# lanl-ansi/Katana.jl

Hardware: AMD Instinct MI355X
Metric: ECP iterations/sec + wall-clock to f_tol=1e-6, 1e5-var synthetic convex NLP (higher is better)
Workload: dtype f64; 1 GPU; cfg3: n=100000 variables, m_lin=50000 linear rows (8 nnz), m_nl=10000 explog rows (k=32 nnz), seed 0, planted non-degenerate vertex optimum, f_tol=1e-6; parallelism=1 GPU

## Files before the change

katana.jl_amd/csrc/engine.hpp:

```cpp
#pragma once
#include <hip/hip_runtime.h>

#include <algorithm>
#include <chrono>
#include <cstdlib>
#include <cmath>
#include <limits>
#include <map>
#include <string>
#include <vector>

#include <rccl/rccl.h>

#include "common.hpp"
#include "types.hpp"
#include "prims.hpp"

namespace ktn {

static const double kInf = std::numeric_limits<double>::infinity();

static inline int pick_group(double avg_len) {
    int g = 4;
    while (g < 64 && 2 * g <= avg_len) g <<= 1;
// ... 169 lines not shown
    void append_link(int64_t nrows, const int64_t* nl_id_host);
    void append_link_dev(int64_t nrows);
    int64_t* list_heads() { return glists ? d_glast.p : d_lastcut.p; }
    int64_t list_count() const { return glists ? nl_total : m_nl; }
    bool lists_ok() const { return !sharded_rows || glists; }
    DBuf<int64_t> c_ptr, c_cnt;
    DBuf<int32_t> c_row;
    DBuf<double> c_val, c_sval, r_sval;
    DBuf<uint32_t> c_perm, c_perm2;
    DBuf<int32_t> c_row2;
    DBuf<int64_t> c_ptr2, c_off;
    int64_t csc_M = -1, csc_NNZ = 0;
    uint64_t lp_epoch = 1, csc_epoch = 0;
    void csc_merge_appended();
    bool w_shift = false;
    int64_t M_lin = 0;
    DBuf<double> wval, wlo, whi, wc, epi_ref, epi_scal;
    DBuf<unsigned long long> epi_newest;
    const double* Wval() const { return w_shift ? wval.p : lp_val.p; }
    const double* Wlo() const { return w_shift ? wlo.p : lp_lo.p; }
    const double* Whi() const { return w_shift ? whi.p : lp_hi.p; }
    const double* Wc() const { return w_shift ? wc.p : lp_c.p; }
    bool want_shift(int mode) const { return prm.epi_shift != 0 && !obj_linear && mode == 0 && !row_sharded() && n_blocks == 0; }
    void build_working();
    void ensure_matrix(bool shift);
    void epi_dot(const double* x);
    DBuf<uint64_t> k_in, k_out;
    DBuf<uint32_t> p_in, p_out;
    DBuf<char> d_sorttmp;
    DBuf<double> dr_r, dc_r;
    DBuf<ColRec> d_crec;
    DBuf<RowRec> d_rrec;
    DBuf<int2> d_cbl;
    bool packed_on = false;
    int packed_trips = 1;
    DBuf<double> dr2, dc2;
    DBuf<double> dr, dc, statr, statc, ch, lh, uh, loh, hih, xh, yh, x0h, y0h, xth, yth, xbar, pv, pw, box;
    DBuf<double> partials, chk_part, chkout, power_v, power_v0;
    int64_t power_v0_n = -1;
    double* h_chk = nullptr;
    double* h_chk_dev = nullptr;
    int64_t lp_iter_budget = 0, dense_credit = 0, dense_run = 0;
    DBuf<int32_t> ds_W, ds_valid;
    DBuf<double> ds_dense, ds_out;
    DBuf<double> md_Binv, md_hW, md_x, md_lam, md_u, md_d, md_r, md_pv, md_c, md_aug, md_prow, md_fcol;
    int64_t md_since_refactor = 0;
    DBuf<double> md_y;
    uint64_t md_y_version = 0;
    bool mid_true_duals(double* y_out);
    int64_t mid_backoff = 0, mid_backoff_len = 0;
    DBuf<int32_t> md_W, md_pi, md_lost;
    DBuf<MidState> md_st;
    bool md_valid = false;
    int64_t mid_credit = 0, mid_run = 0;
    DBuf<int32_t> d_longrows;
    DBuf<int32_t> d_longcols;
    int64_t n_longc = 0;
    int64_t col_gain_max = 0;
    int64_t col_len_max = -1, col_scan_rows = 0;
    int64_t col_removed_rows = 0;
    void find_long_cols();
    void spmv_cols(const SpMat& AT, const double* v, double* out, hipEvent_t e0 = nullptr, hipEvent_t e1 = nullptr);
    static constexpr int kMaxChunk = 512;
    int64_t n_long = 0;
    static constexpr int64_t kLongRow = 2048;
    int64_t max_row_len = (int64_t)1 << 62;
// ... 310 lines not shown
```

katana.jl_amd/csrc/kernels.hpp:

```cpp
#pragma once
#include <hip/hip_runtime.h>

#include <cstdint>
#include <type_traits>

#include "../../include/katana_hip.h"
#include "types.hpp"

namespace ktn {

constexpr int kKindShift = 29;
constexpr int kColMask = (1 << kKindShift) - 1;

template <int G>
__device__ __forceinline__ double group_sum(double v) {
#pragma unroll
    for (int off = G / 2; off > 0; off >>= 1) v += __shfl_xor(v, off, 64);
    return v;
}
template <int G>
__device__ __forceinline__ double group_max(double v) {
#pragma unroll
    for (int off = G / 2; off > 0; off >>= 1) v = fmax(v, __shfl_xor(v, off, 64));
    return v;
// ... 674 lines not shown
                                                     const int32_t* __restrict__ col, const double* __restrict__ jac,
                                                     const double* __restrict__ g, const double* __restrict__ lb, const double* __restrict__ ub,
                                                     const int64_t* __restrict__ lp_rowptr, int32_t* __restrict__ lp_col,
                                                     double* __restrict__ lp_val, double* __restrict__ lp_lo, double* __restrict__ lp_hi) {
    const int64_t r = (int64_t)blockIdx.x * kBlock + threadIdx.x;
    if (r >= nlin) return;
    const int32_t i = lin_rows[r];
    const int64_t beg = rowptr[i], len = rowptr[i + 1] - beg, dst = lp_rowptr[r];
    double b = g[i];
    for (int64_t e = 0; e < len; ++e) {
        const double jv = jac[beg + e];
        lp_col[dst + e] = col[beg + e];
        lp_val[dst + e] = jv;
        b += -0.0 * jv;
    }
    lp_lo[r] = lb[i] - b;
    lp_hi[r] = ub[i] - b;
}

struct LpRows {
    int64_t* rowptr;
    int32_t* col;
    double* val;
    double* lo;
    double* hi;
    double* y;
};

static __global__ __launch_bounds__(kBlock) void k_compact(NlpDev P, const int32_t* __restrict__ nl_rows, int64_t m_nl,
                                                    const int64_t* __restrict__ flag, const int64_t* __restrict__ rank,
                                                    const int64_t* __restrict__ cnt_scan, const double* __restrict__ bconst,
                                                    int64_t base_row, int64_t base_nnz, LpRows L,
                                                    int32_t* __restrict__ viol_slots, int64_t* __restrict__ last_cut,
                                                    int64_t* __restrict__ cut_prev, int inherit) {
    const int64_t gid = (int64_t)blockIdx.x * kBlock + threadIdx.x;
    if (gid >= m_nl) return;
    if (!flag[gid]) return;
    const int32_t r = nl_rows[gid];
    const int64_t v = rank[gid];
    const int64_t R = base_row + v;
    const int64_t len = P.rowptr[r + 1] - P.rowptr[r];
    L.rowptr[R + 1] = base_nnz + cnt_scan[gid] + len;
    const double b = bconst[r];
    L.lo[R] = P.lb[r] - b;
    L.hi[R] = P.ub[r] - b;
    viol_slots[v] = (int32_t)gid;
    double y0 = 0.0;
    const int64_t prev = last_cut[gid];
    if (inherit && prev >= 0) { y0 = L.y[prev]; L.y[prev] = 0.0; }
    L.y[R] = y0;
    cut_prev[R] = prev;
    last_cut[gid] = R;
}

static __global__ __launch_bounds__(kBlock) void k_append_link(int64_t nrows, int64_t base_row, const int64_t* __restrict__ nl_id,
                                                       int64_t nl_total, int64_t* __restrict__ glast,
                                                       int64_t* __restrict__ cut_prev, double* __restrict__ y, int inherit) {
    const int64_t i = (int64_t)blockIdx.x * kBlock + threadIdx.x;
    if (i >= nrows) return;
    const int64_t R = base_row + i, g = nl_id[i];
    double y0 = 0.0;
    int64_t prev = -1;
    if (g >= 0 && g < nl_total) {
        prev = glast[g];
        if (inherit && prev >= 0) { y0 = y[prev]; y[prev] = 0.0; }
        glast[g] = R;
    }
    y[R] = y0;
    cut_prev[R] = prev;
}

static __global__ __launch_bounds__(kBlock) void k_consolidate(int64_t m_nl, const int64_t* __restrict__ last_cut,
                                                        const int64_t* __restrict__ cut_prev, const double* __restrict__ ax,
                                                        const double* __restrict__ lo, const double* __restrict__ hi,
                                                        const double* __restrict__ dr, double thresh,
                                                        double* __restrict__ y, int32_t* __restrict__ moved) {
    const int64_t s = (int64_t)blockIdx.x * kBlock + threadIdx.x;
    if (s >= m_nl) return;
    int64_t best_u = -1, best_l = -1;
    double res_u = -__builtin_inf(), res_l = -__builtin_inf();
    int ncuts = 0;
    for (int64_t r = last_cut[s]; r >= 0; r = cut_prev[r]) {
        ++ncuts;
        const double ru = ax[r] - hi[r], rl = lo[r] - ax[r];
        if (ru > res_u) { res_u = ru; best_u = r; }
// ... 175 lines not shown
};
constexpr unsigned kChkRowMask = 0x141Fu;
constexpr unsigned kChkColMask = 0x6FE0u;
template <int BLOCK, unsigned MASK, int G = 1>
__device__ __forceinline__ void chk_block_store(ChkAcc& a, double* partials) {
    __shared__ double sh[kChkQ][BLOCK / 64];
    const int lane = threadIdx.x & 63, wv = threadIdx.x >> 6;
#pragma unroll
    for (int off = 32; off >= G; off >>= 1) {
#pragma unroll
        for (int q = 0; q < kChkQ; ++q) {
            if (!((MASK >> q) & 1u)) continue;
            const double o = __shfl_xor(a.s[q], off, 64);
            a.s[q] = (q < 12) ? a.s[q] + o : fmax(a.s[q], o);
        }
    }
    if (lane == 0) {
#pragma unroll
        for (int q = 0; q < kChkQ; ++q)
            if ((MASK >> q) & 1u) sh[q][wv] = a.s[q];
    }
    __syncthreads();
    if (threadIdx.x < kChkQ) {
        const int q = threadIdx.x;
        double v = 0.0;
        if ((MASK >> q) & 1u) {
            v = sh[q][0];
            for (int k = 1; k < BLOCK / 64; ++k) v = (q < 12) ? v + sh[q][k] : fmax(v, sh[q][k]);
        }
        partials[(int64_t)blockIdx.x * kChkQ + q] = v;
    }
}

template <int G, bool UPDATE>
__global__ __launch_bounds__(kBlock) void k_pdhg_x(int64_t n, SpMat AT, const double* __restrict__ y,
                                                   double* __restrict__ x, const double* __restrict__ x0,
                                                   double* __restrict__ xt, double* __restrict__ xbar,
                                                   const double* __restrict__ c, const double* __restrict__ l,
                                                   const double* __restrict__ u, double tau, double w, double rho) {
    const int64_t j = ((int64_t)blockIdx.x * kBlock + threadIdx.x) / G;
    const int lane = threadIdx.x & (G - 1);
    if (j >= n) return;
    const int64_t beg = AT.ptr[j], end = AT.ptr[j + 1];
    const double xv = x[j], cj = c[j], lj = l[j], uj = u[j], x0j = (UPDATE || xbar) ? x0[j] : 0.0;
    double acc = 0.0;
    for (int64_t e = beg + lane; e < end; e += G) acc += AT.val[e] * y[AT.idx[e]];
    acc = group_sum<G>(acc);
    if (lane == 0) {
        const double xtv = prox_x(xv, tau, cj, acc, lj, uj);
        if (UPDATE) { xbar[j] = 2.0 * xtv - xv; x[j] = halpern(w, rho, xtv, xv, x0j); }
        else {
            xt[j] = xtv;
            if (xbar) xbar[j] = halpern(w, rho, xtv, xv, x0j);
        }
    }
}

template <int G, bool UPDATE>
__global__ __launch_bounds__(kBlock) void k_pdhg_x_skip(int64_t n, SpMat AT, const double* __restrict__ y,
                                                        double* __restrict__ x, const double* __restrict__ x0,
                                                        double* __restrict__ xt, double* __restrict__ xbar,
                                                        const double* __restrict__ c, const double* __restrict__ l,
                                                        const double* __restrict__ u, double tau, double w, double rho, int64_t skip_longer) {
    const int64_t j = ((int64_t)blockIdx.x * kBlock + threadIdx.x) / G;
    const int lane = threadIdx.x & (G - 1);
    if (j >= n) return;
// ... 199 lines not shown
}

template <int G>
__global__ __launch_bounds__(kBlock) void k_pdhg_y_chk(int64_t m, SpMat A, const double* __restrict__ xt,
                                                       const double* __restrict__ x, const double* __restrict__ y,
                                                       const double* __restrict__ y0, double* __restrict__ yt,
                                                       const double* __restrict__ lo, const double* __restrict__ hi,
                                                       const double* __restrict__ dr, double sigma, int64_t long_thresh,
                                                       double* __restrict__ partials, double* __restrict__ ynext, double w, double rho) {
    const int64_t i = ((int64_t)blockIdx.x * kBlock + threadIdx.x) / G;
    const int lane = threadIdx.x & (G - 1);
    ChkAcc a; a.init();
    const bool on = i < m;
    const int64_t beg = on ? A.ptr[i] : 0, end = on ? A.ptr[i + 1] : 0;
    const bool mine = on && (end - beg <= long_thresh);
    double yv = 0.0, loi = 0.0, hii = 0.0, y0i = 0.0, dri = 1.0;
    if (mine) { yv = y[i]; loi = lo[i]; hii = hi[i]; y0i = y0[i]; dri = dr[i]; }
    double axt = 0.0, axk = 0.0;
    if (mine)
        for (int64_t e = beg + lane; e < end; e += G) {
            const int c = A.idx[e];
            const double v = A.val[e];
            axt += v * xt[c];
            axk += v * x[c];
        }
    axt = group_sum<G>(axt);
    axk = group_sum<G>(axk);
    if (mine && lane == 0) {
        const double ytv = prox_y(yv, sigma, 2.0 * axt - axk, loi, hii);
        yt[i] = ytv;
        if (ynext) ynext[i] = halpern(w, rho, ytv, yv, y0i);
        chk_row_accumulate(a, ytv, yv, y0i, axt, axk, loi, hii, dri);
    }
    chk_block_store<kBlock, kChkRowMask, G>(a, partials);
}

constexpr int kLongBlock = 1024;
template <bool CHECK>
__global__ __launch_bounds__(kLongBlock) void k_pdhg_y_long(const int32_t* __restrict__ rows, SpMat A,
                                                        const double* __restrict__ xa, const double* __restrict__ xb,
                                                        double* __restrict__ y, const double* __restrict__ y0,
                                                        double* __restrict__ yt, const double* __restrict__ lo,
                                                        const double* __restrict__ hi, const double* __restrict__ dr,
                                                        double sigma, double w, double rho, double* __restrict__ partials) {
    const int64_t i = rows[blockIdx.x];
    const int64_t beg = A.ptr[i], end = A.ptr[i + 1];
    double acc = 0.0, acc2 = 0.0;
    for (int64_t e = beg + threadIdx.x; e < end; e += kLongBlock) {
        const int c = A.idx[e];
        const double v = A.val[e];
        acc += v * xa[c];
        if (CHECK) acc2 += v * xb[c];
    }
    __shared__ double sh[2][kLongBlock / 64];
    double a2[2] = {acc, acc2};
    block_sum<kLongBlock>(a2, sh);
    if (threadIdx.x == 0) {
        const double ax = a2[0], ax2 = a2[1];
        const double yv = y[i];
        if (CHECK) {
            const double ytv = prox_y(yv, sigma, 2.0 * ax - ax2, lo[i], hi[i]);
            yt[i] = ytv;
            ChkAcc a; a.init();
            chk_row_accumulate(a, ytv, yv, y0[i], ax, ax2, lo[i], hi[i], dr[i]);
#pragma unroll
            for (int q = 0; q < kChkQ; ++q) partials[(int64_t)blockIdx.x * kChkQ + q] = a.s[q];
        } else {
// ... 82 lines not shown
}
__device__ __forceinline__ void chk_col_accumulate(ChkAcc& a, double xtv, double xv, double x0v, double aty, double cj, double lj,
                                                   double uj, double dcj) {
    const ChkColTerms t = chk_col_terms(xtv, xv, x0v, aty, cj, lj, uj, dcj);
    a.s[5] += t.dx2;
    a.s[6] += t.pobj;
    a.s[7] += t.dobj;
    a.s[8] += t.dx0sq;
    a.s[9] += t.xt2;
    a.s[13] = fmax(a.s[13], t.dres);
    const double r0 = -aty;
    if (r0 > 0.0) { if (isfinite(lj)) { a.s[10] += lj * r0; a.s[11] += fabs(lj * r0); } else a.s[14] = fmax(a.s[14], r0); }
    else if (r0 < 0.0) { if (isfinite(uj)) { a.s[10] += uj * r0; a.s[11] += fabs(uj * r0); } else a.s[14] = fmax(a.s[14], -r0); }
}
template <int G>
__global__ __launch_bounds__(kBlock) void k_chk_cols(int64_t n, SpMat AT, const double* __restrict__ x,
                                                     const double* __restrict__ xt, const double* __restrict__ x0,
                                                     const double* __restrict__ yt, const double* __restrict__ c,
                                                     const double* __restrict__ l, const double* __restrict__ u,
                                                     const double* __restrict__ dc, double* __restrict__ partials) {
    const int64_t j = ((int64_t)blockIdx.x * kBlock + threadIdx.x) / G;
    const int lane = threadIdx.x & (G - 1);
    ChkAcc a; a.init();
    const bool on = j < n;
    const int64_t beg = on ? AT.ptr[j] : 0, end = on ? AT.ptr[j + 1] : 0;
    double xtv = 0.0, xv = 0.0, x0v = 0.0, cj = 0.0, lj = 0.0, uj = 0.0, dcj = 1.0;
    if (on) { xtv = xt[j]; xv = x[j]; x0v = x0[j]; cj = c[j]; lj = l[j]; uj = u[j]; dcj = dc[j]; }
    double aty = 0.0;
    for (int64_t e = beg + lane; e < end; e += G) aty += AT.val[e] * yt[AT.idx[e]];
    aty = group_sum<G>(aty);
    if (on && lane == 0) {
        chk_col_accumulate(a, xtv, xv, x0v, aty, cj, lj, uj, dcj);
    }
    chk_block_store<kBlock, kChkColMask, G>(a, partials);
}

template <bool UPDATE>
__global__ __launch_bounds__(kBlock) void k_x_prox(int64_t n, const double* __restrict__ aty, double* __restrict__ x,
                                                   const double* __restrict__ x0, double* __restrict__ xt, double* __restrict__ xbar,
                                                   const double* __restrict__ c, const double* __restrict__ l,
                                                   const double* __restrict__ u, double tau, double w, double rho) {
    const int64_t j = (int64_t)blockIdx.x * kBlock + threadIdx.x;
    if (j >= n) return;
    const double xv = x[j];
    const double xtv = prox_x(xv, tau, c[j], aty[j], l[j], u[j]);
    if (UPDATE) { xbar[j] = 2.0 * xtv - xv; x[j] = halpern(w, rho, xtv, xv, x0[j]); }
    else xt[j] = xtv;
}
static __global__ __launch_bounds__(kBlock) void k_chk_cols_vec(int64_t n, const double* __restrict__ atyv, const double* __restrict__ x,
                                                         const double* __restrict__ xt, const double* __restrict__ x0,
                                                         const double* __restrict__ c, const double* __restrict__ l,
                                                         const double* __restrict__ u, const double* __restrict__ dc,
                                                         double* __restrict__ partials) {
    const int64_t j = (int64_t)blockIdx.x * kBlock + threadIdx.x;
    ChkAcc a; a.init();
    if (j < n) {
        const double xtv = xt[j], xv = x[j], x0v = x0[j], cj = c[j], lj = l[j], uj = u[j], dcj = dc[j], aty = atyv[j];
        chk_col_accumulate(a, xtv, xv, x0v, aty, cj, lj, uj, dcj);
    }
    chk_block_store<kBlock, kChkColMask>(a, partials);
}

__device__ __forceinline__ double ipc_load(const double* p) {
    return __longlong_as_double((long long)__hip_atomic_load((unsigned long long*)p, __ATOMIC_RELAXED, __HIP_MEMORY_SCOPE_SYSTEM));
}
static __global__ __launch_bounds__(64) void k_ipc_barrier(IpcPeers P, int rank, int world, unsigned long long epoch, long long timeout_ticks,
                                                    int* __restrict__ err) {
// ... 657 lines not shown
    if (i < n) out[i] = (s > 0.0) ? a[i] / sqrt(s) : 0.0;
}
static __global__ __launch_bounds__(kBlock) void k_fill(int64_t n, double* __restrict__ z, double v) {
    const int64_t i = (int64_t)blockIdx.x * kBlock + threadIdx.x;
    if (i < n) z[i] = v;
}
static __global__ __launch_bounds__(kBlock) void k_axpy_scaled(int64_t n, const double* __restrict__ a, double s, double* __restrict__ out) {
    const int64_t i = (int64_t)blockIdx.x * kBlock + threadIdx.x;
    if (i < n) out[i] = a[i] * s;
}

template <int G>
__global__ __launch_bounds__(kBlock) void k_csc_keys(int64_t m, const int64_t* __restrict__ rowptr,
                                                     const int32_t* __restrict__ col, uint64_t* __restrict__ keys,
                                                     uint32_t* __restrict__ vals, int64_t* __restrict__ colcount) {
    const int64_t i = ((int64_t)blockIdx.x * kBlock + threadIdx.x) / G;
    const int lane = threadIdx.x & (G - 1);
    if (i >= m) return;
    for (int64_t e = rowptr[i] + lane; e < rowptr[i + 1]; e += G) {
        const uint32_t c = (uint32_t)col[e];
        keys[e] = ((uint64_t)c << 32) | (uint64_t)(uint32_t)i;
        vals[e] = (uint32_t)e;
        atomicAdd(reinterpret_cast<unsigned long long*>(&colcount[c]), 1ULL);
    }
}
static __global__ __launch_bounds__(kBlock) void k_cscm_count(int64_t e0, int64_t nnz, const int32_t* __restrict__ col, int64_t* __restrict__ cnt) {
    const int64_t e = e0 + (int64_t)blockIdx.x * kBlock + threadIdx.x;
    if (e < nnz) atomicAdd(reinterpret_cast<unsigned long long*>(&cnt[col[e]]), 1ULL);
}
template <int G>
__global__ __launch_bounds__(kBlock) void k_cscm_move(int64_t n, const int64_t* __restrict__ old_ptr, const int64_t* __restrict__ off,
                                                      const int32_t* __restrict__ old_row, const uint32_t* __restrict__ old_perm,
                                                      int64_t* __restrict__ new_ptr, int32_t* __restrict__ new_row,
                                                      uint32_t* __restrict__ new_perm) {
    const int64_t j = ((int64_t)blockIdx.x * kBlock + threadIdx.x) / G;
    const int lane = threadIdx.x & (G - 1);
    if (j > n) return;
    if (j == n) { if (lane == 0) new_ptr[n] = old_ptr[n] + off[n]; return; }
    const int64_t src = old_ptr[j], len = old_ptr[j + 1] - src, dst = src + off[j];
    for (int64_t k = lane; k < len; k += G) { new_row[dst + k] = old_row[src + k]; new_perm[dst + k] = old_perm[src + k]; }
    if (lane == 0) new_ptr[j] = dst;
}
template <int G>
__global__ __launch_bounds__(kBlock) void k_cscm_place(int64_t m0, int64_t m, const int64_t* __restrict__ rowptr, const int32_t* __restrict__ col,
                                                       const int64_t* __restrict__ old_ptr, const int64_t* __restrict__ off,
                                                       int64_t* __restrict__ cursor, int32_t* __restrict__ new_row,
                                                       uint32_t* __restrict__ new_perm) {
    const int64_t r = m0 + ((int64_t)blockIdx.x * kBlock + threadIdx.x) / G;
    const int lane = threadIdx.x & (G - 1);
    if (r >= m) return;
    for (int64_t e = rowptr[r] + lane; e < rowptr[r + 1]; e += G) {
        const int32_t j = col[e];
        const int64_t k = (int64_t)atomicAdd(reinterpret_cast<unsigned long long*>(&cursor[j]), 1ULL);
        const int64_t pos = old_ptr[j + 1] + off[j] + k;
        new_row[pos] = (int32_t)r;
        new_perm[pos] = (uint32_t)e;
    }
}
static __global__ __launch_bounds__(kBlock) void k_cscm_order(int64_t n, const int64_t* __restrict__ old_ptr, const int64_t* __restrict__ off,
                                                       int32_t* __restrict__ new_row, uint32_t* __restrict__ new_perm) {
    const int64_t j = (int64_t)blockIdx.x * kBlock + threadIdx.x;
    if (j >= n) return;
    const int64_t cnt = off[j + 1] - off[j];
    if (cnt < 2) return;
    const int64_t b = old_ptr[j + 1] + off[j];
    for (int64_t a = 1; a < cnt; ++a) {
        const int32_t rr = new_row[b + a];
        const uint32_t pp = new_perm[b + a];
        int64_t q = a - 1;
        while (q >= 0 && (new_row[b + q] > rr || (new_row[b + q] == rr && new_perm[b + q] > pp))) {
// ... 213 lines not shown
```

katana.jl_amd/csrc/lp.hip:

```cpp
#include "engine.hpp"
#include "launch.hpp"
#include "kernels.hpp"
#include "pdhg_check.hpp"
#include "dense_lp.hpp"
#include "mid_lp.hpp"
#include "batch_lp.hpp"

namespace ktn {

double Engine::dev_dot(int64_t n, const double* a, const double* b) {
    hipLaunchKernelGGL(k_dot_partial, dim3(kRedBlocks), dim3(kBlock), 0, stream, n, a, b, partials.p);
    hipLaunchKernelGGL(k_sum_final, dim3(1), dim3(kRedBlocks), 0, stream, partials.p, kRedBlocks, chkout.p + 2 * kChkQ);
    double v = 0.0;
    KTN_HIP(hipMemcpyAsync(&v, chkout.p + 2 * kChkQ, sizeof(double), hipMemcpyDeviceToHost, stream));
    sync();
    return v;
}

double Engine::dev_finite_sq(int64_t n, const double* a) {
    hipLaunchKernelGGL(k_finite_sq_partial, dim3(kRedBlocks), dim3(kBlock), 0, stream, n, a, partials.p);
    hipLaunchKernelGGL(k_sum_final, dim3(1), dim3(kRedBlocks), 0, stream, partials.p, kRedBlocks, chkout.p + 2 * kChkQ);
    double v = 0.0;
    KTN_HIP(hipMemcpyAsync(&v, chkout.p + 2 * kChkQ, sizeof(double), hipMemcpyDeviceToHost, stream));
    sync();
// ... 310 lines not shown
    const bool tiled_chk_off = dev.no_tiled_check;
    if (tiled_on && m > 0 && !tiled_chk_off) {
        const int64_t brow_t = ceil_div(m, (int64_t)kBlock), bcol_t = ceil_div(n, (int64_t)kBlock);
        launch_tiled(tAT, n, m, yh.p, nullptr);
        if (row_sharded()) {
            LAUNCH_1(k_tile_vec, n, stream, n, tAT.pcnt.p, tpart.p, pv.p);
            allreduce(pv.p, (size_t)n, 0);
            LAUNCH_1(k_x_prox<false>, n, stream, n, pv.p, xh.p, x0h.p, xth.p, xbar.p, ch.p, lh.p, uh.p, tau, 0.0, 1.0);
        } else {
            LAUNCH_1(k_x_epilogue_chk, n, stream, n, tAT.pcnt.p, tpart.p, xh.p, xth.p, ch.p, lh.p, uh.p, tau);
        }
        launch_tiled(tA, m, n, xth.p, nullptr);
        LAUNCH_1(k_tile_vec, m, stream, m, tA.pcnt.p, tpart.p, pw.p);
        launch_tiled(tA, m, n, xh.p, nullptr);
        LAUNCH_1(k_y_epilogue_chk, m, stream, m, tA.pcnt.p, tpart.p, pw.p, (n_long > 0 ? A.ptr : (const int64_t*)nullptr), thr, yh.p, y0h.p,
                 yth.p, loh.p, hih.p, dr.p, sigma, prow);
        if (n_long > 0)
            hipLaunchKernelGGL((k_pdhg_y_long<true>), dim3((unsigned)n_long), dim3(kLongBlock), 0, stream, d_longrows.p, A, xth.p, xh.p,
                               yh.p, y0h.p, yth.p, loh.p, hih.p, dr.p, sigma, 0.0, 1.0, prow + (size_t)brow_t * kChkQ);
        chk_nrow = (int)(brow_t + n_long);
        launch_tiled(tAT, n, m, yth.p, nullptr);
        LAUNCH_1(k_tile_vec, n, stream, n, tAT.pcnt.p, tpart.p, pv.p);
        if (row_sharded()) allreduce(pv.p, (size_t)n, 0);
        LAUNCH_1(k_chk_cols_vec, n, stream, n, pv.p, xh.p, xth.p, x0h.p, ch.p, lh.p, uh.p, dc.p, pcol);
        chk_ncol = (int)bcol_t;
        hipLaunchKernelGGL(k_chk_final, dim3(2 * kChkQ), dim3(kRedBlocks), 0, stream, prow, chk_nrow, pcol, chk_ncol, chk_target());
        if (row_sharded()) {
            allreduce(chkout.p, 12, 0);
            allreduce(chkout.p + 12, 4, 1);
        }
        return false;
    }
    const bool spec = w_next >= 0.0 && m > 0 && !row_sharded() && n_long == 0 && n_longc == 0;
    if (spec) {
        xnext.resize((size_t)n, stream); ynext.resize((size_t)m, stream);
        LAUNCH_GB(grp_cols, k_pdhg_x, false, n, stream, n, AT, yh.p, xh.p, x0h.p, xth.p, xnext.p, ch.p, lh.p, uh.p, tau, w_next, rho);
    } else {
        launch_x(AT, tau, 0.0, 1.0, false, nullptr, nullptr);
    }
    if (m > 0) {
        LAUNCH_G(grp_rows, k_pdhg_y_chk, m, stream, m, A, xth.p, xh.p, yh.p, y0h.p, yth.p, loh.p, hih.p, dr.p, sigma, thr, prow,
                 spec ? ynext.p : (double*)nullptr, w_next, rho);
        if (n_long > 0)
            hipLaunchKernelGGL((k_pdhg_y_long<true>), dim3((unsigned)n_long), dim3(kLongBlock), 0, stream, d_longrows.p, A, xth.p, xh.p,
                               yh.p, y0h.p, yth.p, loh.p, hih.p, dr.p, sigma, 0.0, 1.0, prow + (size_t)brow * kChkQ);
    }
    chk_nrow = (m > 0) ? (int)(brow + n_long) : 0;
    if (row_sharded() || n_longc > 0) {
        if (m == 0) LAUNCH_1(k_fill, n, stream, n, pv.p, 0.0);
        spmv_cols(AT, yth.p, pv.p);
        allreduce(pv.p, (size_t)n, 0);
        chk_ncol = ceil_div(n, kBlock);
        LAUNCH_1(k_chk_cols_vec, n, stream, n, pv.p, xh.p, xth.p, x0h.p, ch.p, lh.p, uh.p, dc.p, pcol);
    } else {
        LAUNCH_G(grp_cols, k_chk_cols, n, stream, n, AT, xh.p, xth.p, x0h.p, yth.p, ch.p, lh.p, uh.p, dc.p, pcol);
        chk_ncol = (int)bcol;
    }
    hipLaunchKernelGGL(k_chk_final, dim3(2 * kChkQ), dim3(kRedBlocks), 0, stream, prow, chk_nrow, pcol, chk_ncol, chk_target());
    if (row_sharded()) {
        allreduce(chkout.p, 12, 0);
        allreduce(chkout.p + 12, 4, 1);
    }
    return spec;
}

LpResult Engine::lp_solve(double tol_p, double tol_g, int mode, bool identity_scaling) {
    md_y_version = 0;
    const bool dense_ok = mode == 0 && !identity_scaling && !row_sharded() && prm.lp_dense_after != 0 && n_lp >= 1 && n_lp <= kDenseMaxN &&
                          M * n_lp <= 8000000;
    const bool mid_ok = mode == 0 && !identity_scaling && !row_sharded() && prm.lp_dense_after != 0 && n_lp > kDenseMaxN &&
                        n_lp <= std::min<int64_t>(prm.lp_mid_max_var, kMidMaxN) && n_blocks == 0 && M < ((int64_t)1 << 29);
    if (mid_ok && mid_backoff > 0) {
        --mid_backoff;
    } else if (mid_ok) {
        auto failed = [&]() {
            stats["mid_lp_fallbacks"] += 1.0;
            mid_credit = 0;
            mid_backoff_len = std::min<int64_t>(2 * std::max<int64_t>(mid_backoff_len, 4), 256);
            mid_backoff = mid_backoff_len;
        };
        if (prm.lp_dense_after < 0 || mid_credit > 0) {
            if (mid_credit > 0) --mid_credit;
            LpResult R;
            if (lp_solve_mid(&R)) return R;
            failed();
            return lp_solve_core(tol_p, tol_g, mode, identity_scaling);
        }
        lp_iter_budget = prm.lp_dense_after;
// ... 263 lines not shown
        const int64_t units_t = ceil_div(M, (int64_t)kTileOut) * ceil_div(n_lp, (int64_t)kTileIn);
        const int64_t units_tt = ceil_div(n_lp, (int64_t)kTileOut) * ceil_div(M, (int64_t)kTileIn);
        tiled_on = prm.lp_tiled_nnz > 0 && NNZ >= prm.lp_tiled_nnz && n_lp >= 2 * kTileIn && M >= 2 * kTileIn &&
                   NNZ >= 4096 * std::max(units_t, units_tt);
        if (tenv) tiled_on = dev.tiled != 0 && M > 0 && NNZ > 0;
        if (same_matrix) tiled_on = tiled_built;
        else if (tiled_on) {
            auto tt = std::chrono::steady_clock::now();
            tiled_on = build_tiled(tA, M, n_lp, lp_rowptr.p, lp_col.p, r_sval.p, kLongRow) &&
                       build_tiled(tAT, n_lp, M, c_ptr.p, c_row.p, c_sval.p, (int64_t)1 << 62);
            tpart.resize((size_t)std::max<int64_t>(tA.pieces * M, tAT.pieces * n_lp), stream);
            stats["lp_tiled_builds"] += 1.0;
            stats["lp_tiled_build_time_s"] += std::chrono::duration<double>(std::chrono::steady_clock::now() - tt).count();
            if (!tiled_on) stats["lp_tiled_overflows"] += 1.0;
        }
        tiled_built = tiled_on;
    }
}

void Engine::lp_resize_iterates() {
    const size_t n = (size_t)n_lp, mm = (size_t)std::max<int64_t>(M, 1);
    ch.resize(n, stream); lh.resize(n, stream); uh.resize(n, stream); xh.resize(n, stream);
    x0h.resize(n, stream); xth.resize(n, stream); xbar.resize(n, stream); pv.resize(n, stream);
    loh.resize(mm, stream); hih.resize(mm, stream); yh.resize(mm, stream); y0h.resize(mm, stream);
    yth.resize(mm, stream); pw.resize(mm, stream);
}

void Engine::lp_set_anchors(bool want_packed) {
    const int64_t n = n_lp, m = M;
    const size_t mm = (size_t)std::max<int64_t>(m, 1);
    packed_on = want_packed && !tiled_on && !row_sharded() && NNZ < ((int64_t)1 << 31) && !dev.no_packed;
    if (dev.packed_trips > 0) packed_trips = dev.packed_trips;
    if (packed_on) {
        d_crec.resize((size_t)n, stream); d_cbl.resize((size_t)n, stream); d_rrec.resize(mm, stream);
        LAUNCH_1(k_pack_both, std::max(n, m), stream, n, c_ptr.p, ch.p, lh.p, uh.p, xh.p, x0h.p, d_crec.p, d_cbl.p,
                 m, lp_rowptr.p, loh.p, hih.p, yh.p, y0h.p, d_rrec.p);
    } else {
        KTN_HIP(hipMemcpyAsync(x0h.p, xh.p, n * sizeof(double), hipMemcpyDeviceToDevice, stream));
        if (m > 0) KTN_HIP(hipMemcpyAsync(y0h.p, yh.p, m * sizeof(double), hipMemcpyDeviceToDevice, stream));
    }
}

void Engine::lp_read_check(double* q) {
    if (chk_pinned()) {
        sync();
        std::memcpy(q, h_chk, 2 * kChkQ * sizeof(double));
    } else {
        KTN_HIP(hipMemcpyAsync(q, chkout.p, 2 * kChkQ * sizeof(double), hipMemcpyDeviceToHost, stream));
        sync();
        ipc_check();
    }
}

void Engine::lp_restart() {
    const int64_t n = n_lp, m = M;
    LAUNCH_1(k_restart_set, std::max(n, m), stream, n, m, xth.p, xh.p, x0h.p, yth.p, yh.p, y0h.p, packed_on ? d_crec.p : (ColRec*)nullptr,
             packed_on ? d_rrec.p : (RowRec*)nullptr);
}

void Engine::lp_advance(bool spec, int64_t k, double rho) {
    const int64_t n = n_lp, m = M;
    if (spec) {
        xh.swap(xnext); yh.swap(ynext);
    } else {
        const double w = (double)(k + 1) / (double)(k + 2);
        LAUNCH_1(k_halpern2, std::max(n, m), stream, n, m, xh.p, xth.p, x0h.p, yh.p, yth.p, y0h.p, w, rho);
    }
// ... 480 lines not shown
```

katana.jl_amd/csrc/pool.hip:

```cpp
#include "engine.hpp"
#include "launch.hpp"
#include "kernels.hpp"
#include "mid_lp.hpp"

namespace ktn {

LpRows Engine::lp_view() {
    LpRows L;
    L.rowptr = lp_rowptr.p; L.col = lp_col.p; L.val = lp_val.p; L.lo = lp_lo.p; L.hi = lp_hi.p; L.y = lp_y.p;
    return L;
}

void Engine::append_link(int64_t nrows, const int64_t* nl_id_host) {
    d_nlid.upload(nl_id_host, (size_t)nrows, stream);
    LAUNCH_1(k_append_link, nrows, stream, nrows, M, d_nlid.p, nl_total, d_glast.p, d_cutprev.p, lp_y.p, (int)prm.lp_dual_inherit);
    check_launch();
}

void Engine::append_link_dev(int64_t nrows) {
    LAUNCH_1(k_append_link, nrows, stream, nrows, M, d_nlid.p, nl_total, d_glast.p, d_cutprev.p, lp_y.p, (int)prm.lp_dual_inherit);
    check_launch();
}

void Engine::pack_rows_launch(int64_t nr, int64_t nz, int64_t first_row, int64_t base, bool ids, int64_t id_offset, double* dev_out) {
    LAUNCH_1(k_pack_rows, std::max(nr, nz), stream, nr, nz, lp_rowptr.p + first_row, lp_col.p + base, lp_val.p + base,
             lp_lo.p + first_row, lp_hi.p + first_row, ids ? (const int32_t*)d_violslots.p : (const int32_t*)nullptr,
             id_offset, dev_out);
    check_launch();
}
void Engine::unpack_rows_launch(int64_t nrows, int64_t nnz, const double* dev_in) {
    LAUNCH_1(k_unpack_rows, std::max(nrows, nnz), stream, nrows, nnz, dev_in, NNZ, n_lp, lp_rowptr.p + M + 1, lp_col.p + NNZ,
             lp_val.p + NNZ, lp_lo.p + M, lp_hi.p + M, d_nlid.p, d_anynf.p + 1);
    check_launch();
}

void Engine::reserve_lp(int64_t rows, int64_t nnz) {
    const size_t r = (size_t)rows + 1, z = (size_t)nnz + 1;
    for (DBuf<double>* b : {&lp_lo, &lp_hi, &lp_y, &lp_lo2, &lp_hi2, &lp_y2, &dr, &dr2, &statr, &loh, &hih, &yh, &y0h, &yth, &pw}) b->reserve(r, stream);
    for (DBuf<int64_t>* b : {&lp_rowptr, &lp_rowptr2, &d_cutprev, &d_cutprev2, &d_keep, &d_keepnnz, &d_newidx, &d_newptr}) b->reserve(r, stream);
    for (DBuf<int32_t>* b : {&d_age, &d_age2, &d_longrows}) b->reserve(r, stream);
    for (DBuf<double>* b : {&lp_val, &lp_val2, &c_val, &c_sval, &r_sval}) b->reserve(z, stream);
    for (DBuf<int32_t>* b : {&lp_col, &lp_col2, &c_row, &c_row2}) b->reserve(z, stream);
    c_perm.reserve(z, stream); c_perm2.reserve(z, stream);
    k_in.reserve(z, stream); k_out.reserve(z, stream); p_in.reserve(z, stream); p_out.reserve(z, stream);
    d_rrec.reserve(r, stream);
    d_crec.reserve((size_t)n_lp + 1, stream); d_cbl.reserve((size_t)n_lp + 1, stream);
    chk_part.reserve((r / 4 + (size_t)n_lp / 4 + 4096) * kChkQ, stream);
    d_sorttmp.reserve(sort_pairs_temp_bytes(z) + 16, stream);
    d_scantmp.reserve(scan_i64_temp_bytes(std::max(r, (size_t)n_lp + 2)) + 16, stream);
}

void Engine::rebuild_csc() {
    const bool no_merge = dev.no_csc_merge;
    c_val.resize((size_t)NNZ + 1, stream);
    const int64_t ranks = !sharded_rows ? 1 : (glists && m_nl > 0 ? (nl_total + m_nl - 1) / m_nl : 8);
    const bool few_per_col = col_gain_max * ranks <= 128;
    if (!no_merge && n_longc == 0 && few_per_col && csc_epoch == lp_epoch && csc_M >= 0 && M >= csc_M && NNZ >= csc_NNZ && NNZ < ((int64_t)1 << 32)) {
        if (M > csc_M) csc_merge_appended();
        stats["lp_csc_merges"] += 1.0;
    } else {
        c_ptr.resize((size_t)n_lp + 1, stream);
        c_cnt.resize((size_t)n_lp + 1, stream);
        c_cnt.zero(stream);
        c_row.resize((size_t)NNZ + 1, stream);
        c_perm.resize((size_t)NNZ + 1, stream);
        if (NNZ > 0) {
            k_in.resize((size_t)NNZ, stream); k_out.resize((size_t)NNZ, stream);
            p_in.resize((size_t)NNZ, stream); p_out.resize((size_t)NNZ, stream);
            LAUNCH_G(pick_group((double)NNZ / (double)std::max<int64_t>(M, 1)), k_csc_keys, M, stream, M, lp_rowptr.p, lp_col.p, k_in.p,
                     p_in.p, c_cnt.p);
            check_launch();
        }
        exclusive_scan(c_cnt.p, c_ptr.p, (size_t)n_lp + 1);
        if (NNZ > 0) {
            int bits = 1;
            while (((int64_t)1 << bits) < n_lp + 1 && bits < 31) ++bits;
            size_t need = sort_pairs_temp_bytes((size_t)NNZ);
            d_sorttmp.resize(need + 16, stream);
            KTN_HIP(sort_pairs_u64_u32(d_sorttmp.p, need, k_in.p, k_out.p, p_in.p, p_out.p, (size_t)NNZ, 32, 32 + bits, stream));
// ... 18 lines not shown
    d_longcols.resize((size_t)n_lp, stream);
    KTN_HIP(hipMemsetAsync(d_anynf.p + 1, 0, 2 * sizeof(int32_t), stream));
    LAUNCH_1(k_find_long_max, n_lp, stream, n_lp, c_ptr.p, kLongRow, d_longcols.p, d_anynf.p + 1);
    int32_t r[2] = {0, 0};
    KTN_HIP(hipMemcpyAsync(r, d_anynf.p + 1, 8, hipMemcpyDeviceToHost, stream));
    sync();
    n_longc = r[0];
    col_len_max = r[1];
    col_scan_rows = M;
    stats["lp_long_col_scans"] += 1.0;
    stats["lp_long_cols"] = (double)n_longc;
    stats["lp_long_cols_max"] = std::max(stats["lp_long_cols_max"], (double)n_longc);
    if (n_longc > 1) {
        std::vector<int32_t> tmp((size_t)n_longc);
        KTN_HIP(hipMemcpyAsync(tmp.data(), d_longcols.p, (size_t)n_longc * sizeof(int32_t), hipMemcpyDeviceToHost, stream));
        sync();
        std::sort(tmp.begin(), tmp.end());
        KTN_HIP(hipMemcpyAsync(d_longcols.p, tmp.data(), (size_t)n_longc * sizeof(int32_t), hipMemcpyHostToDevice, stream));
        sync();
    }
}

void Engine::csc_merge_appended() {
    const int64_t n = n_lp, nnz_new = NNZ - csc_NNZ;
    c_off.resize((size_t)n + 1, stream);
    c_cnt.resize((size_t)n + 1, stream);
    c_cnt.zero(stream);
    LAUNCH_1(k_cscm_count, nnz_new, stream, csc_NNZ, NNZ, lp_col.p, c_cnt.p);
    exclusive_scan(c_cnt.p, c_off.p, (size_t)n + 1);
    c_ptr2.resize((size_t)n + 1, stream);
    c_row2.resize((size_t)NNZ + 1, stream);
    c_perm2.resize((size_t)NNZ + 1, stream);
    const int gc = pick_group((double)csc_NNZ / (double)std::max<int64_t>(n, 1));
    LAUNCH_G(gc, k_cscm_move, n + 1, stream, n, c_ptr.p, c_off.p, c_row.p, c_perm.p, c_ptr2.p, c_row2.p, c_perm2.p);
    c_cnt.zero(stream);
    LAUNCH_G(pick_group((double)nnz_new / (double)std::max<int64_t>(M - csc_M, 1)), k_cscm_place, M - csc_M, stream, csc_M, M, lp_rowptr.p, lp_col.p, c_ptr.p,
             c_off.p, c_cnt.p, c_row2.p, c_perm2.p);
    LAUNCH_1(k_cscm_order, n, stream, n, c_ptr.p, c_off.p, c_row2.p, c_perm2.p);
    check_launch();
    c_ptr.swap(c_ptr2); c_row.swap(c_row2); c_perm.swap(c_perm2);
}

void Engine::ensure_matrix(bool shift) {
    if (shift != w_shift) { lp_dirty = true; ++lp_version; }
    if (!lp_dirty) return;
    w_shift = shift;
    if (shift) build_working();
    rebuild_csc();
}

void Engine::build_working() {
    const int32_t tcol = (int32_t)n0;
    const size_t mm = (size_t)std::max<int64_t>(M, 1);
    wval.resize((size_t)NNZ + 1, stream); wlo.resize(mm, stream); whi.resize(mm, stream);
    wc.resize((size_t)n_lp, stream); epi_ref.resize((size_t)n_lp, stream); epi_scal.resize(2, stream); epi_newest.resize(1, stream);
    if (NNZ > 0) KTN_HIP(hipMemcpyAsync(wval.p, lp_val.p, (size_t)NNZ * sizeof(double), hipMemcpyDeviceToDevice, stream));
    if (M > 0) {
        KTN_HIP(hipMemcpyAsync(wlo.p, lp_lo.p, (size_t)M * sizeof(double), hipMemcpyDeviceToDevice, stream));
        KTN_HIP(hipMemcpyAsync(whi.p, lp_hi.p, (size_t)M * sizeof(double), hipMemcpyDeviceToDevice, stream));
    }
    epi_ref.zero(stream); epi_scal.zero(stream); epi_newest.zero(stream);
    const int64_t rows = M - M_lin;
    LAUNCH_1(k_epi_newest, rows, stream, M_lin, M, lp_rowptr.p, lp_col.p, tcol, epi_newest.p);
    if (rows > 0) {
        hipLaunchKernelGGL(k_epi_setref, dim3(64), dim3(kBlock), 0, stream, epi_newest.p, lp_rowptr.p, lp_col.p, lp_val.p, lp_lo.p, lp_hi.p,
                           tcol, epi_ref.p, epi_scal.p);
        hipLaunchKernelGGL(k_epi_shift, dim3((unsigned)(rows * kEpiChunks)), dim3(kBlock), 0, stream, M_lin, M, lp_rowptr.p, lp_col.p,
                           lp_val.p, lp_lo.p, lp_hi.p, tcol, epi_ref.p, epi_scal.p, wval.p, wlo.p, whi.p);
// ... 117 lines not shown
```

katana.jl_amd/csrc/sweep.hip:

```cpp
#include <cstring>
#include <unordered_map>

#include "engine.hpp"
#include "launch.hpp"
#include "kernels.hpp"
#include "tape_classes.hpp"
#include "quad_rows.hpp"
#include "batch_lp.hpp"
#include "batch_ecp.hpp"
#include "dense_lp.hpp"

namespace ktn {

static void postfix_to_nodes(const int32_t* op, const double* arg, int64_t len, const int32_t* rcols, int64_t rlen,
                             int64_t jac_base, std::vector<int64_t>& slot_of, std::vector<int32_t>& nop,
                             std::vector<int32_t>& na, std::vector<int32_t>& nb, std::vector<double>& nc) {
    std::vector<int32_t> st;
    const int64_t base = (int64_t)nop.size();
    for (int64_t s = rlen - 1; s >= 0; --s) slot_of[(size_t)rcols[s]] = s;
    struct Reset {
        std::vector<int64_t>& m; const int32_t* c; int64_t n;
        ~Reset() { for (int64_t s = 0; s < n; ++s) m[(size_t)c[s]] = -1; }
    } reset{slot_of, rcols, rlen};
    for (int64_t t = 0; t < len; ++t) {
// ... 1031 lines not shown
    if (cap > 0 && V > cap && !anynf) {
        d_dkeys.resize((size_t)m_nl, stream); d_dsorted.resize((size_t)m_nl, stream);
        LAUNCH_1(k_depth_keys, m_nl, stream, P, d_nlrows.p, m_nl, d_g.p, d_flag.p, d_dkeys.p);
        const size_t need = sort_keys_desc_temp_bytes((size_t)m_nl);
        d_sorttmp.resize(need + 16, stream);
        KTN_HIP(sort_keys_desc_u64(d_sorttmp.p, need, d_dkeys.p, d_dsorted.p, (size_t)m_nl, stream));
        LAUNCH_1(k_depth_reflag, m_nl, stream, m_nl, d_dkeys.p, d_dsorted.p, cap, d_flag.p, d_cnt.p);
        check_launch();
        exclusive_scan(d_flag.p, d_rank.p, (size_t)m_nl);
        exclusive_scan(d_cnt.p, d_cntscan.p, (size_t)m_nl);
        KTN_HIP(hipMemcpyAsync(&tail[0], d_flag.p + (m_nl - 1), 8, hipMemcpyDeviceToHost, stream));
        KTN_HIP(hipMemcpyAsync(&tail[1], d_rank.p + (m_nl - 1), 8, hipMemcpyDeviceToHost, stream));
        KTN_HIP(hipMemcpyAsync(&tail[2], d_cnt.p + (m_nl - 1), 8, hipMemcpyDeviceToHost, stream));
        KTN_HIP(hipMemcpyAsync(&tail[3], d_cntscan.p + (m_nl - 1), 8, hipMemcpyDeviceToHost, stream));
        sync();
        V = tail[0] + tail[1];
        nnzV = tail[2] + tail[3];
        stats["cut_selections"] += 1.0;
        stats["cuts_skipped"] += (double)(*nviol_out - V);
    }
    if (anynf) {
        std::fprintf(stderr, "WARNING: Nonlinear constraint or objective likely undefined within domain\n");
        *nonfinite_out = true;
        return;
    }
    if (V > 0) {
        if (esh_mode()) esh_search(d_x, f_tol);
        lp_rowptr.resize((size_t)(M + V + 1), stream);
        lp_lo.resize((size_t)(M + V), stream);
        lp_hi.resize((size_t)(M + V), stream);
        lp_y.resize((size_t)(M + V), stream);
        d_cutprev.resize((size_t)(M + V), stream);
        d_age.resize((size_t)(M + V), stream);
        KTN_HIP(hipMemsetAsync(d_age.p + M, 0, (size_t)V * sizeof(int32_t), stream));
        lp_col.resize((size_t)(NNZ + nnzV), stream);
        lp_val.resize((size_t)(NNZ + nnzV), stream);
        d_violslots.resize((size_t)V, stream);
        LpRows L = lp_view();
        LAUNCH_1(k_compact, m_nl, stream, P, d_nlrows.p, m_nl, d_flag.p, d_rank.p, d_cntscan.p, d_bconst.p, M, NNZ, L,
                 d_violslots.p, d_lastcut.p, d_cutprev.p, (int)(prm.lp_dual_inherit && !glists));
        if (esh_mode()) esh_emit(d_x, V);
        else LAUNCH_G(grp_sweep, k_emit, V, stream, P, d_nlrows.p, d_violslots.p, V, d_x, d_jac.p, d_maxc.p,
                      prm.cut_coef_rng, 1, M, L);
        check_launch();
        M += V;
        NNZ += nnzV;
        numcuts += V;
        last_sweep_cuts = V;
        lp_dirty = true; ++lp_version;
    }
    sync();
    stats["sep_time_s"] += std::chrono::duration<double>(std::chrono::steady_clock::now() - t0).count();
}

void Engine::global_sweep(const double* d_x, double f_tol, int64_t* nviol, double* maxviol, bool* nonfinite) {
    sweep(d_x, f_tol, nviol, maxviol, nonfinite);
    if (!row_sharded()) return;
    double v[2] = {(double)*nviol, *nonfinite ? 1.0 : 0.0};
    allreduce_host(v, 2, 0);
    double mv = *maxviol;
    allreduce_host(&mv, 1, 1);
    *nviol = (int64_t)(v[0] + 0.5);
    *nonfinite = v[1] > 0.0;
    *maxviol = mv;
}

}
```

Baseline: 344.2 ECP iterations/s.

## Add packed check kernels, group-aware block reduction, and fold memsets into kernels

Adds packed-record variants of the PDHG x, y and column-check kernels. They read column and row metadata from packed structs and store (xt, x) as interleaved double2, so the row SpMV fetches both values with one gather. It also replaces the per-block partial-sum store with a version that writes only group leaders to shared memory and reduces in one wavefront. The age memset and the cursor zeroing are folded into existing kernels, and the host sync at the end of the sweep is skipped unless profiling or row-sharded. Dropping the sync may change timing attribution in stats, and the packed path adds an extra double2 buffer write per column.

```diff
diff --git a/katana.jl_amd/csrc/engine.hpp b/katana.jl_amd/csrc/engine.hpp
--- a/katana.jl_amd/csrc/engine.hpp
+++ b/katana.jl_amd/csrc/engine.hpp
@@ -225,6 +225,7 @@
     DBuf<ColRec> d_crec;
     DBuf<RowRec> d_rrec;
     DBuf<int2> d_cbl;
+    DBuf<double2> d_xtx;
     bool packed_on = false;
     int packed_trips = 1;
     DBuf<double> dr2, dc2;
diff --git a/katana.jl_amd/csrc/kernels.hpp b/katana.jl_amd/csrc/kernels.hpp
--- a/katana.jl_amd/csrc/kernels.hpp
+++ b/katana.jl_amd/csrc/kernels.hpp
@@ -730,7 +730,7 @@
                                                     const int64_t* __restrict__ cnt_scan, const double* __restrict__ bconst,
                                                     int64_t base_row, int64_t base_nnz, LpRows L,
                                                     int32_t* __restrict__ viol_slots, int64_t* __restrict__ last_cut,
-                                                    int64_t* __restrict__ cut_prev, int inherit) {
+                                                    int64_t* __restrict__ cut_prev, int32_t* __restrict__ age, int inherit) {
     const int64_t gid = (int64_t)blockIdx.x * kBlock + threadIdx.x;
     if (gid >= m_nl) return;
     if (!flag[gid]) return;
@@ -749,6 +749,7 @@
     L.y[R] = y0;
     cut_prev[R] = prev;
     last_cut[gid] = R;
+    age[R] = 0;
 }
 
 static __global__ __launch_bounds__(kBlock) void k_append_link(int64_t nrows, int64_t base_row, const int64_t* __restrict__ nl_id,
@@ -990,6 +991,41 @@
     }
 }
 
+template <int BLOCK, unsigned MASK, int G>
+__device__ __forceinline__ void chk_block_store_groups(ChkAcc& a, double* partials) {
+    const int lane = threadIdx.x & 63, wv = threadIdx.x >> 6;
+    static_assert(BLOCK == 256 && kChkQ == 16, "lane (k, q) of the first wavefront: four wavefronts x sixteen quantities");
+    constexpr int L = 64 / G, NQ = __builtin_popcount(MASK);
+    __shared__ double sh[BLOCK / 64][L][NQ];
+    if ((lane & (G - 1)) == 0) {
+        int s = 0;
+#pragma unroll
+        for (int q = 0; q < kChkQ; ++q)
+            if ((MASK >> q) & 1u) sh[wv][lane / G][s++] = a.s[q];
+    }
+    __syncthreads();
+    if (wv == 0) {
+        const int q = lane & 15, k = lane >> 4;
+        const bool live = (MASK >> q) & 1u;
+        const int s = live ? __builtin_popcount(MASK & ((1u << q) - 1u)) : 0;
+        double v[L];
+#pragma unroll
+        for (int i = 0; i < L; ++i) v[i] = live ? sh[k][i][s] : 0.0;
+#pragma unroll
+        for (int h = L / 2; h > 0; h >>= 1) {
+#pragma unroll
+            for (int i = 0; i < h; ++i) v[i] = (q < 12) ? v[i] + v[i + h] : fmax(v[i], v[i + h]);
+        }
+        double r = __shfl(v[0], q, 64);
+#pragma unroll
+        for (int kk = 1; kk < BLOCK / 64; ++kk) {
+            const double o = __shfl(v[0], q + 16 * kk, 64);
+            r = (q < 12) ? r + o : fmax(r, o);
+        }
+        if (lane < kChkQ) partials[(int64_t)blockIdx.x * kChkQ + q] = r;
+    }
+}
+
 template <int G, bool UPDATE>
 __global__ __launch_bounds__(kBlock) void k_pdhg_x(int64_t n, SpMat AT, const double* __restrict__ y,
                                                    double* __restrict__ x, const double* __restrict__ x0,
@@ -1255,7 +1291,7 @@
         if (ynext) ynext[i] = halpern(w, rho, ytv, yv, y0i);
         chk_row_accumulate(a, ytv, yv, y0i, axt, axk, loi, hii, dri);
     }
-    chk_block_store<kBlock, kChkRowMask, G>(a, partials);
+    chk_block_store_groups<kBlock, kChkRowMask, G>(a, partials);
 }
 
 constexpr int kLongBlock = 1024;
@@ -1404,7 +1440,84 @@
     if (on && lane == 0) {
         chk_col_accumulate(a, xtv, xv, x0v, aty, cj, lj, uj, dcj);
     }
-    chk_block_store<kBlock, kChkColMask, G>(a, partials);
+    chk_block_store_groups<kBlock, kChkColMask, G>(a, partials);
+}
+
+template <int G>
+__global__ __launch_bounds__(kBlock) void k_pdhg_x_chk_packed(int64_t n, const int2* __restrict__ bl, const int32_t* __restrict__ idx,
+                                                              const double* __restrict__ val, const double* __restrict__ y,
+                                                              const double* __restrict__ x, double* __restrict__ xt,
+                                                              double2* __restrict__ xtx, double* __restrict__ xnext,
+                                                              const ColRec* __restrict__ rec, double tau, double w, double rho) {
+    const int64_t j = ((int64_t)blockIdx.x * kBlock + threadIdx.x) / G;
+    const int lane = threadIdx.x & (G - 1);
+    if (j >= n) return;
+    const int2 b = bl[j];
+    const ColRec r = rec[j];
+    const double xv = x[j];
+    double acc = 0.0;
+    for (int e = b.x + lane; e < b.x + b.y; e += G) acc += val[e] * y[idx[e]];
+    acc = group_sum<G>(acc);
+    if (lane == 0) {
+        const double xtv = prox_x(xv, tau, r.c, acc, r.l, r.u);
+        xt[j] = xtv;
+        xtx[j] = make_double2(xtv, xv);
+        if (xnext) xnext[j] = halpern(w, rho, xtv, xv, r.x0);
+    }
+}
+template <int G>
+__global__ __launch_bounds__(kBlock) void k_pdhg_y_chk_packed(int64_t m, const int32_t* __restrict__ idx, const double* __restrict__ val,
+                                                              const double2* __restrict__ xtx, const double* __restrict__ y, double* __restrict__ yt,
+                                                              const RowRec* __restrict__ rec, const double* __restrict__ dr,
+                                                              double sigma, int long_thresh, double* __restrict__ partials,
+                                                              double* __restrict__ ynext, double w, double rho) {
+    const int64_t i = ((int64_t)blockIdx.x * kBlock + threadIdx.x) / G;
+    const int lane = threadIdx.x & (G - 1);
+    ChkAcc a; a.init();
+    const bool on = i < m;
+    RowRec r; r.lo = 0.0; r.hi = 0.0; r.y0 = 0.0; r.beg = 0; r.len = 0;
+    if (on) r = rec[i];
+    const bool mine = on && r.len <= long_thresh;
+    double yv = 0.0, dri = 1.0;
+    if (mine) { yv = y[i]; dri = dr[i]; }
+    double axt = 0.0, axk = 0.0;
+    if (mine)
+        for (int e = r.beg + lane; e < r.beg + r.len; e += G) {
+            const double v = val[e];
+            const double2 p = xtx[idx[e]];
+            axt += v * p.x;
+            axk += v * p.y;
+        }
+    axt = group_sum<G>(axt);
+    axk = group_sum<G>(axk);
+    if (mine && lane == 0) {
+        const double ytv = prox_y(yv, sigma, 2.0 * axt - axk, r.lo, r.hi);
+        yt[i] = ytv;
+        if (ynext) ynext[i] = halpern(w, rho, ytv, yv, r.y0);
+        chk_row_accumulate(a, ytv, yv, r.y0, axt, axk, r.lo, r.hi, dri);
+    }
+    chk_block_store_groups<kBlock, kChkRowMask, G>(a, partials);
+}
+template <int G>
+__global__ __launch_bounds__(kBlock) void k_chk_cols_packed(int64_t n, const int2* __restrict__ bl, const int32_t* __restrict__ idx,
+                                                            const double* __restrict__ val, const double2* __restrict__ xtx,
+                                                            const double* __restrict__ yt, const ColRec* __restrict__ rec,
+                                                            const double* __restrict__ dc, double* __restrict__ partials) {
+    const int64_t j = ((int64_t)blockIdx.x * kBlock + threadIdx.x) / G;
+    const int lane = threadIdx.x & (G - 1);
+    ChkAcc a; a.init();
+    const bool on = j < n;
+    const int2 b = on ? bl[j] : make_int2(0, 0);
+    ColRec r; r.c = 0.0; r.l = 0.0; r.u = 0.0; r.x0 = 0.0;
+    double xtv = 0.0, xv = 0.0, dcj = 1.0;
+    if (on) { r = rec[j]; const double2 p = xtx[j]; xtv = p.x; xv = p.y; dcj = dc[j]; }
+    double aty = 0.0;
+    for (int e = b.x + lane; e < b.x + b.y; e += G) aty += val[e] * yt[idx[e]];
+    aty = group_sum<G>(aty);
+    if (on && lane == 0) {
+        chk_col_accumulate(a, xtv, xv, r.x0, aty, r.c, r.l, r.u, dcj);
+    }
+    chk_block_store_groups<kBlock, kChkColMask, G>(a, partials);
 }
 
 template <bool UPDATE>
@@ -2128,10 +2241,11 @@
 __global__ __launch_bounds__(kBlock) void k_cscm_move(int64_t n, const int64_t* __restrict__ old_ptr, const int64_t* __restrict__ off,
                                                       const int32_t* __restrict__ old_row, const uint32_t* __restrict__ old_perm,
                                                       int64_t* __restrict__ new_ptr, int32_t* __restrict__ new_row,
-                                                      uint32_t* __restrict__ new_perm) {
+                                                      uint32_t* __restrict__ new_perm, int64_t* __restrict__ cursor) {
     const int64_t j = ((int64_t)blockIdx.x * kBlock + threadIdx.x) / G;
     const int lane = threadIdx.x & (G - 1);
     if (j > n) return;
+    if (lane == 0) cursor[j] = 0;
     if (j == n) { if (lane == 0) new_ptr[n] = old_ptr[n] + off[n]; return; }
     const int64_t src = old_ptr[j], len = old_ptr[j + 1] - src, dst = src + off[j];
     for (int64_t k = lane; k < len; k += G) { new_row[dst + k] = old_row[src + k]; new_perm[dst + k] = old_perm[src + k]; }
diff --git a/katana.jl_amd/csrc/lp.hip b/katana.jl_amd/csrc/lp.hip
--- a/katana.jl_amd/csrc/lp.hip
+++ b/katana.jl_amd/csrc/lp.hip
@@ -366,15 +366,23 @@
         return false;
     }
     const bool spec = w_next >= 0.0 && m > 0 && !row_sharded() && n_long == 0 && n_longc == 0;
+    const bool packed_chk = packed_on && n_longc == 0;
     if (spec) {
         xnext.resize((size_t)n, stream); ynext.resize((size_t)m, stream);
-        LAUNCH_GB(grp_cols, k_pdhg_x, false, n, stream, n, AT, yh.p, xh.p, x0h.p, xth.p, xnext.p, ch.p, lh.p, uh.p, tau, w_next, rho);
+        if (packed_chk) LAUNCH_G(grp_cols, k_pdhg_x_chk_packed, n, stream, n, d_cbl.p, AT.idx, AT.val, yh.p, xh.p, xth.p, d_xtx.p, xnext.p, d_crec.p, tau, w_next, rho);
+        else LAUNCH_GB(grp_cols, k_pdhg_x, false, n, stream, n, AT, yh.p, xh.p, x0h.p, xth.p, xnext.p, ch.p, lh.p, uh.p, tau, w_next, rho);
+    } else if (packed_chk) {
+        LAUNCH_G(grp_cols, k_pdhg_x_chk_packed, n, stream, n, d_cbl.p, AT.idx, AT.val, yh.p, xh.p, xth.p, d_xtx.p, (double*)nullptr, d_crec.p, tau, 0.0, 1.0);
     } else {
         launch_x(AT, tau, 0.0, 1.0, false, nullptr, nullptr);
     }
     if (m > 0) {
-        LAUNCH_G(grp_rows, k_pdhg_y_chk, m, stream, m, A, xth.p, xh.p, yh.p, y0h.p, yth.p, loh.p, hih.p, dr.p, sigma, thr, prow,
-                 spec ? ynext.p : (double*)nullptr, w_next, rho);
+        if (packed_chk)
+            LAUNCH_G(grp_rows, k_pdhg_y_chk_packed, m, stream, m, A.idx, A.val, d_xtx.p, yh.p, yth.p, d_rrec.p, dr.p, sigma,
+                     n_long > 0 ? (int)kLongRow : 0x7fffffff, prow, spec ? ynext.p : (double*)nullptr, w_next, rho);
+        else
+            LAUNCH_G(grp_rows, k_pdhg_y_chk, m, stream, m, A, xth.p, xh.p, yh.p, y0h.p, yth.p, loh.p, hih.p, dr.p, sigma, thr, prow,
+                     spec ? ynext.p : (double*)nullptr, w_next, rho);
         if (n_long > 0)
             hipLaunchKernelGGL((k_pdhg_y_long<true>), dim3((unsigned)n_long), dim3(kLongBlock), 0, stream, d_longrows.p, A, xth.p, xh.p,
                                yh.p, y0h.p, yth.p, loh.p, hih.p, dr.p, sigma, 0.0, 1.0, prow + (size_t)brow * kChkQ);
@@ -387,7 +395,8 @@
         chk_ncol = ceil_div(n, kBlock);
         LAUNCH_1(k_chk_cols_vec, n, stream, n, pv.p, xh.p, xth.p, x0h.p, ch.p, lh.p, uh.p, dc.p, pcol);
     } else {
-        LAUNCH_G(grp_cols, k_chk_cols, n, stream, n, AT, xh.p, xth.p, x0h.p, yth.p, ch.p, lh.p, uh.p, dc.p, pcol);
+        if (packed_chk) LAUNCH_G(grp_cols, k_chk_cols_packed, n, stream, n, d_cbl.p, AT.idx, AT.val, d_xtx.p, yth.p, d_crec.p, dc.p, pcol);
+        else LAUNCH_G(grp_cols, k_chk_cols, n, stream, n, AT, xh.p, xth.p, x0h.p, yth.p, ch.p, lh.p, uh.p, dc.p, pcol);
         chk_ncol = (int)bcol;
     }
     hipLaunchKernelGGL(k_chk_final, dim3(2 * kChkQ), dim3(kRedBlocks), 0, stream, prow, chk_nrow, pcol, chk_ncol, chk_target());
@@ -717,7 +726,7 @@
     packed_on = want_packed && !tiled_on && !row_sharded() && NNZ < ((int64_t)1 << 31) && !dev.no_packed;
     if (dev.packed_trips > 0) packed_trips = dev.packed_trips;
     if (packed_on) {
-        d_crec.resize((size_t)n, stream); d_cbl.resize((size_t)n, stream); d_rrec.resize(mm, stream);
+        d_crec.resize((size_t)n, stream); d_cbl.resize((size_t)n, stream); d_rrec.resize(mm, stream); d_xtx.resize((size_t)n, stream);
         LAUNCH_1(k_pack_both, std::max(n, m), stream, n, c_ptr.p, ch.p, lh.p, uh.p, xh.p, x0h.p, d_crec.p, d_cbl.p,
                  m, lp_rowptr.p, loh.p, hih.p, yh.p, y0h.p, d_rrec.p);
     } else {
diff --git a/katana.jl_amd/csrc/pool.hip b/katana.jl_amd/csrc/pool.hip
--- a/katana.jl_amd/csrc/pool.hip
+++ b/katana.jl_amd/csrc/pool.hip
@@ -44,7 +44,7 @@
     c_perm.reserve(z, stream); c_perm2.reserve(z, stream);
     k_in.reserve(z, stream); k_out.reserve(z, stream); p_in.reserve(z, stream); p_out.reserve(z, stream);
     d_rrec.reserve(r, stream);
-    d_crec.reserve((size_t)n_lp + 1, stream); d_cbl.reserve((size_t)n_lp + 1, stream);
+    d_crec.reserve((size_t)n_lp + 1, stream); d_cbl.reserve((size_t)n_lp + 1, stream); d_xtx.reserve((size_t)n_lp + 1, stream);
     chk_part.reserve((r / 4 + (size_t)n_lp / 4 + 4096) * kChkQ, stream);
     d_sorttmp.reserve(sort_pairs_temp_bytes(z) + 16, stream);
     d_scantmp.reserve(scan_i64_temp_bytes(std::max(r, (size_t)n_lp + 2)) + 16, stream);
@@ -129,8 +129,7 @@
     c_row2.resize((size_t)NNZ + 1, stream);
     c_perm2.resize((size_t)NNZ + 1, stream);
     const int gc = pick_group((double)csc_NNZ / (double)std::max<int64_t>(n, 1));
-    LAUNCH_G(gc, k_cscm_move, n + 1, stream, n, c_ptr.p, c_off.p, c_row.p, c_perm.p, c_ptr2.p, c_row2.p, c_perm2.p);
-    c_cnt.zero(stream);
+    LAUNCH_G(gc, k_cscm_move, n + 1, stream, n, c_ptr.p, c_off.p, c_row.p, c_perm.p, c_ptr2.p, c_row2.p, c_perm2.p, c_cnt.p);
     LAUNCH_G(pick_group((double)nnz_new / (double)std::max<int64_t>(M - csc_M, 1)), k_cscm_place, M - csc_M, stream, csc_M, M, lp_rowptr.p, lp_col.p, c_ptr.p,
              c_off.p, c_cnt.p, c_row2.p, c_perm2.p);
     LAUNCH_1(k_cscm_order, n, stream, n, c_ptr.p, c_off.p, c_row2.p, c_perm2.p);
diff --git a/katana.jl_amd/csrc/sweep.hip b/katana.jl_amd/csrc/sweep.hip
--- a/katana.jl_amd/csrc/sweep.hip
+++ b/katana.jl_amd/csrc/sweep.hip
@@ -1087,13 +1087,12 @@
         lp_y.resize((size_t)(M + V), stream);
         d_cutprev.resize((size_t)(M + V), stream);
         d_age.resize((size_t)(M + V), stream);
-        KTN_HIP(hipMemsetAsync(d_age.p + M, 0, (size_t)V * sizeof(int32_t), stream));
         lp_col.resize((size_t)(NNZ + nnzV), stream);
         lp_val.resize((size_t)(NNZ + nnzV), stream);
         d_violslots.resize((size_t)V, stream);
         LpRows L = lp_view();
         LAUNCH_1(k_compact, m_nl, stream, P, d_nlrows.p, m_nl, d_flag.p, d_rank.p, d_cntscan.p, d_bconst.p, M, NNZ, L,
-                 d_violslots.p, d_lastcut.p, d_cutprev.p, (int)(prm.lp_dual_inherit && !glists));
+                 d_violslots.p, d_lastcut.p, d_cutprev.p, d_age.p, (int)(prm.lp_dual_inherit && !glists));
         if (esh_mode()) esh_emit(d_x, V);
         else LAUNCH_G(grp_sweep, k_emit, V, stream, P, d_nlrows.p, d_violslots.p, V, d_x, d_jac.p, d_maxc.p,
                       prm.cut_coef_rng, 1, M, L);
@@ -1104,7 +1103,7 @@
         last_sweep_cuts = V;
         lp_dirty = true; ++lp_version;
     }
-    sync();
+    if (prm.profile || row_sharded()) sync();
     stats["sep_time_s"] += std::chrono::duration<double>(std::chrono::steady_clock::now() - t0).count();
 }
 
```

Result: faster. 351.7 ECP iterations/s (median of 4 runs) (+2.2%).
